# Haochen-Wang409/U2PL

Hardware: AMD Instinct MI355X
Metric: train images/sec at 769x769 (R101-DeepLabv3+) (higher is better)
Workload: dtype f32

## Files before the change

include/u2pl_hip.h:

```cpp
#ifndef U2PL_HIP_H
#define U2PL_HIP_H

#include <stddef.h>
#include <stdint.h>

#ifdef __cplusplus
extern "C" {
#endif

#ifndef __HIP_PLATFORM_AMD__
typedef struct ihipStream_t* hipStream_t;
#endif

#define U2PL_SEL_MAX_SLOTS 8
#define U2PL_SEL_WORD_NVALID 0
#define U2PL_SEL_WORD_NTOTAL 1
#define U2PL_SEL_WORD_VAL 40
#define U2PL_SEL_WORD_THR 56

int u2pl_bilinear_up_f32(const float* in, long sn, long sc, long sh, long sw, int N, int C, int h, int w,
                         float* out_nchw, int H, int W, hipStream_t stream);
int u2pl_bilinear_up_bwd_f32(const float* gout_nchw, int N, int C, int H, int W, float* gin, long sn, long sc,
                             long sh, long sw, int h, int w, hipStream_t stream);
int u2pl_pseudo_label_f32(const float* logits_nchw, int N, int C, int H, int W, float* conf, long long* label,
// ... 136 lines not shown
                          int accumulate, int N, int Hin, int Win, int Cin, int Hout, int Wout, int Cout, int R,
                          int S, int stride, int pad, int dil, hipStream_t stream);
int u2pl_wgrad_set_tr(int on);
int u2pl_im2col_f32(const float* x, long ldx, float* col, int Kp, int N, int Hin, int Win, int Cin, int Hout,
                    int Wout, int R, int S, int stride, int pad, int dil, hipStream_t stream);

size_t u2pl_weight_split3_bytes(int rows, int K, int batch);
int u2pl_weight_split3_f32(const float* w, long zw, int rows, int K, int batch, void* out, hipStream_t stream);
int u2pl_weight_split3_multi_f32(const void* jobs, int njobs, long total, hipStream_t stream);
int u2pl_weight_split3_pad_rows(int rows);
int u2pl_wino_weight_multi_f32(const void* jobs, int njobs, long total, hipStream_t stream);
int u2pl_igemm_ws_stat_blocks(int N, int Hout, int Wout);
int u2pl_igemm_ws_set_persist(int on);
int u2pl_conv2d_fwd_ws_f32(const float* x, long ldx, const void* wsplit, const float* bias, float* y, long ldy, int N,
                           int Hin, int Win, int Cin, int Hout, int Wout, int Cout, int R, int S, int stride, int pad,
                           int dil, hipStream_t stream);
int u2pl_conv2d_fwd_bnstats_ws_f32(const float* x, long ldx, const void* wsplit, const float* bias, float* y, long ldy,
                                   int N, int Hin, int Win, int Cin, int Hout, int Wout, int Cout, int R, int S,
                                   int stride, int pad, int dil, const float* pivot, float* stats_partial,
                                   hipStream_t stream);
int u2pl_conv2d_fwd_bnact_ws_f32(const float* x, long ldx, const void* wsplit, const float* bias, float* y, long ldy, int N,
                                 int Hin, int Win, int Cin, int Hout, int Wout, int Cout, int R, int S, int stride,
                                 int pad, int dil, const float* mean, const float* invstd, const float* gamma,
                                 const float* beta, const float* res, long ldr, int relu, hipStream_t stream);
int u2pl_conv2d_dgrad_ws_f32(const float* dy, long lddy, const void* wTsplit, float* dx, long lddx, int N, int Hin,
                             int Win, int Cin, int Hout, int Wout, int Cout, int R, int S, int stride, int pad, int dil,
                             hipStream_t stream);
int u2pl_gemm_batched_ws_f32(const float* x, long ldx, long zx, const void* wsplit, float* y, long ldy, long zy, long M,
                             int K, int Nn, int batch, hipStream_t stream);

size_t u2pl_weight_split2h_bytes(int rows, int K, int batch);
int u2pl_weight_split2h_f32(const float* w, long zw, int rows, int K, int batch, void* out, void* job_scratch, hipStream_t stream);
int u2pl_weight_split2h_multi_f32(const void* jobs, int njobs, long total, hipStream_t stream);
int u2pl_amax_words(void);
int u2pl_absmax_f32(const float* x, long ld, long M, int C, float* out, int clear, hipStream_t stream);
int u2pl_bn_apply_amax_f32(const float* x, long ldx, const float* mean, const float* invstd, const float* gamma, const float* beta,
                           const float* res, long ldr, int relu, const float* drop, long rows_per_image, float* y, long ldy, long M,
                           int C, float* y_amax, hipStream_t stream);
int u2pl_bn_bwd_apply_amax_f32(const float* dy, long lddy, const float* x, long ldx, const float* y, long ldy, const float* mean,
                               const float* invstd, const float* gamma, const float* drop, long rows_per_image, const double* sums,
                               double count, float* dx, long lddx, float* dres, long lddr, long M, int C, const double* psums,
                               float* gsink, float* bsink, int accumulate, float* dx_amax, float* dres_amax, const float* relu_beta,
                               hipStream_t stream);
int u2pl_bn_bwd_sums_mx_f32(const float* dy, long lddy, const float* x, long ldx, const float* mean, const float* invstd,
                            const float* gamma, const float* beta, const float* drop, long rows_per_image, long M, int C,
                            void* workspace, double* sums, hipStream_t stream);
int u2pl_wino_input_amax_f32(const float* x, long ldx, int N, int H, int W, int C, int dil, int mt, float* V, float* v_amax,
                             hipStream_t stream);
int u2pl_wino_output_bnact_amax_f32(const float* Mb, int N, int H, int W, int O, int dil, int mt, const float* bias, float* y,
                                    long ldy, const float* mean, const float* invstd, const float* gamma, const float* beta,
                                    const float* res, long ldr, int relu, float* y_amax, hipStream_t stream);
int u2pl_wino_gy_amax_f32(const float* gy, long ldg, int N, int H, int W, int O, int dil, int mt, float* Mg, float* mg_amax,
                          hipStream_t stream);
int u2pl_conv2d_fwd_wsh_f32(const float* x, long ldx, const float* x_amax, const void* wsplit, const float* bias, float* y, long ldy,
                            int N, int Hin, int Win, int Cin, int Hout, int Wout, int Cout, int R, int S, int stride, int pad,
                            int dil, hipStream_t stream);
int u2pl_conv2d_fwd_bnstats_wsh_f32(const float* x, long ldx, const float* x_amax, const void* wsplit, const float* bias, float* y,
                                    long ldy, int N, int Hin, int Win, int Cin, int Hout, int Wout, int Cout, int R, int S,
                                    int stride, int pad, int dil, const float* pivot, float* stats_partial, hipStream_t stream);
int u2pl_conv2d_fwd_bnact_wsh_f32(const float* x, long ldx, const float* x_amax, const void* wsplit, const float* bias, float* y,
                                  long ldy, int N, int Hin, int Win, int Cin, int Hout, int Wout, int Cout, int R, int S,
                                  int stride, int pad, int dil, const float* mean, const float* invstd, const float* gamma,
                                  const float* beta, const float* res, long ldr, int relu, float* y_amax, hipStream_t stream);
int u2pl_conv2d_dgrad_wsh_f32(const float* dy, long lddy, const float* dy_amax, const void* wTsplit, float* dx, long lddx, int N,
                              int Hin, int Win, int Cin, int Hout, int Wout, int Cout, int R, int S, int stride, int pad, int dil,
                              hipStream_t stream);
// ... 92 lines not shown
```

u2pl_amd/csrc/igemm_ws.hip:

```cpp
#include <stdlib.h>
#include <type_traits>
#include "common.h"
#include "conv_geom.h"
#include "u2pl_hip.h"

template <int B, int E, class F>
__device__ __forceinline__ void static_for(F&& f) {
    if constexpr (B < E) {
        f(std::integral_constant<int, B>{});
        static_for<B + 1, E>(f);
    }
}

#define WS_ROW_B 64
__host__ __device__ static inline int ws_pad_rows(int rows) { return rows <= 128 ? 128 : (rows + 255) & ~255; }

__global__ void k_weight_split3(const float* __restrict__ w, long zw, unsigned short* __restrict__ out, long zo, int rows,
                                int Np, int K) {
    w += (long)blockIdx.y * zw;
    out += (long)blockIdx.y * zo;
    const int nseg = K / 8;
    const long total = (long)Np * nseg;
    for (long i = blockIdx.x * (long)blockDim.x + threadIdx.x; i < total; i += (long)gridDim.x * blockDim.x) {
        const int sg = (int)(i % nseg), n = (int)(i / nseg);
        float4 v0 = make_float4(0.f, 0.f, 0.f, 0.f), v1 = v0;
        if (n < rows) {
            const float4* src = (const float4*)(w + (long)n * K + sg * 8);
            v0 = src[0];
            v1 = src[1];
        }
        uint2 a0, a1, a2, b0, b1, b2;
        split3_bf16(v0, a0, a1, a2);
        split3_bf16(v1, b0, b1, b2);
        const int c = sg >> 2, s = sg & 3;
        const long base = (((long)c * 3) * Np + n) * 32 + ((s ^ ((n >> 2) & 3)) << 3);
        const long pl = (long)Np * 32;
        *(uint4*)(out + base) = make_uint4(a0.x, a0.y, b0.x, b0.y);
// ... 46 lines not shown
        split3_bf16(v1, b0, b1, b2);
        const int c = sg >> 2, s = sg & 3;
        const long pl = (long)j.Np * 32;
        unsigned short* out = j.out + (long)z * (j.K / 32) * 3 * pl;
        const long base = (((long)c * 3) * j.Np + n) * 32 + ((s ^ ((n >> 2) & 3)) << 3);
        *(uint4*)(out + base) = make_uint4(a0.x, a0.y, b0.x, b0.y);
        *(uint4*)(out + base + pl) = make_uint4(a1.x, a1.y, b1.x, b1.y);
        *(uint4*)(out + base + 2 * pl) = make_uint4(a2.x, a2.y, b2.x, b2.y);
    }
}
U2PL_API int u2pl_weight_split3_multi_f32(const void* jobs, int njobs, long total, hipStream_t stream) {
    if (njobs <= 0 || total <= 0) return njobs == 0 ? 0 : U2PL_EINVAL;
    U2PL_LAUNCH(k_weight_split3_multi, dim3(grid_for(total, 256, 4096)), dim3(256), 0, stream, (const SplitJob*)jobs, njobs, total);
    U2PL_LAUNCH_CHECK();
    return 0;
}
U2PL_API int u2pl_weight_split3_pad_rows(int rows) { return ws_pad_rows(rows); }

U2PL_API size_t u2pl_weight_split3_bytes(int rows, int K, int batch) {
    return (size_t)batch * (K / 32) * 3 * ws_pad_rows(rows) * WS_ROW_B;
}
U2PL_API int u2pl_weight_split3_f32(const float* w, long zw, int rows, int K, int batch, void* out, hipStream_t stream) {
    if (rows <= 0 || K <= 0 || (K % 32) || batch <= 0) return U2PL_EINVAL;
    const int Np = ws_pad_rows(rows);
    const long total = (long)Np * (K / 8);
    dim3 grid(grid_for(total, 256, 2048), batch);
    U2PL_LAUNCH(k_weight_split3, grid, dim3(256), 0, stream, w, zw, (unsigned short*)out,
                (long)(u2pl_weight_split3_bytes(rows, K, 1) / 2), rows, Np, K);
    U2PL_LAUNCH_CHECK();
    return 0;
}

__host__ __device__ static inline size_t ws2_plane_bytes(int Np, int K, int batch) { return (size_t)batch * (K / 32) * 2 * Np * WS_ROW_B; }
__global__ void k_weight_amax_clear(const SplitJob* __restrict__ jobs, int njobs) {
    const int t = blockIdx.x * blockDim.x + threadIdx.x;
    if (t >= njobs) return;
    const SplitJob j = jobs[t];
    unsigned* slot = (unsigned*)((char*)j.out + ws2_plane_bytes(j.Np, j.K, j.batch));
    for (int z = 0; z < ((j.batch + 3) & ~3); ++z) slot[z] = 0u;
}
#define WS_AMAX_SPAN 8192
__global__ __launch_bounds__(256) void k_weight_absmax_multi(const SplitJob* __restrict__ jobs, int njobs, long total) {
    const long begin = (long)blockIdx.x * WS_AMAX_SPAN, end = begin + WS_AMAX_SPAN < total ? begin + WS_AMAX_SPAN : total;
    unsigned* slot = nullptr;
    unsigned m = 0u;
    int lo = 0;
    SplitJob j = jobs[0];
    bool have = false;
    for (long i = begin + threadIdx.x; i < end; i += 256) {
        if (!have || i < j.seg_begin || i >= j.seg_begin + (long)j.batch * j.Np * (j.K / 8)) {
            lo = 0;
            int hi = njobs - 1;
            while (lo < hi) {
                const int mid = (lo + hi + 1) >> 1;
                if (jobs[mid].seg_begin <= i) lo = mid; else hi = mid - 1;
            }
            j = jobs[lo];
            have = true;
        }
        const int nseg = j.K / 8;
        const long per = (long)j.Np * nseg;
        long r = i - j.seg_begin;
        const int z = (int)(r / per);
        r -= (long)z * per;
        unsigned* sl = (unsigned*)((char*)j.out + ws2_plane_bytes(j.Np, j.K, j.batch)) + z;
        if (sl != slot) {
            if (slot && m) atomicMax(slot, m);
            slot = sl;
            m = 0u;
        }
        const int n = (int)(r / nseg), sg = (int)(r % nseg);
        if (n < j.rows) {
            const float4* src = (const float4*)(j.src + ((long)z * j.rows + n) * j.K + sg * 8);
            m = amax_bits4(amax_bits4(m, src[0]), src[1]);
        }
    }
    const unsigned long long key = (unsigned long long)slot;
    const unsigned long long first = (unsigned)__builtin_amdgcn_readfirstlane((int)(unsigned)key) |
                                     ((unsigned long long)(unsigned)__builtin_amdgcn_readfirstlane((int)(unsigned)(key >> 32)) << 32);
    if (__all(key == first)) {
        m = wave_max_u(m);
        if ((threadIdx.x & 63) == 0 && slot && m) atomicMax(slot, m);
    } else if (slot && m) {
        atomicMax(slot, m);
    }
}
__global__ __launch_bounds__(256) void k_weight_split2h_multi(const SplitJob* __restrict__ jobs, int njobs, long total) {
    const long begin = (long)blockIdx.x * WS_AMAX_SPAN, end = begin + WS_AMAX_SPAN < total ? begin + WS_AMAX_SPAN : total;
    SplitJob j = jobs[0];
    bool have = false;
    for (long i = begin + threadIdx.x; i < end; i += 256) {
        if (!have || i < j.seg_begin || i >= j.seg_begin + (long)j.batch * j.Np * (j.K / 8)) {
            int lo = 0, hi = njobs - 1;
            while (lo < hi) {
                const int mid = (lo + hi + 1) >> 1;
                if (jobs[mid].seg_begin <= i) lo = mid; else hi = mid - 1;
            }
            j = jobs[lo];
            have = true;
        }
        const int nseg = j.K / 8;
        const long per = (long)j.Np * nseg;
        long r = i - j.seg_begin;
        const int z = (int)(r / per);
        r -= (long)z * per;
        int sg, n;
        float4 v0 = make_float4(0.f, 0.f, 0.f, 0.f), v1 = v0;
        if (j.kind == 0) {
            sg = (int)(r % nseg);
            n = (int)(r / nseg);
            if (n < j.rows) {
                const float4* src = (const float4*)(j.src + ((long)z * j.rows + n) * j.K + sg * 8);
                v0 = src[0];
                v1 = src[1];
            }
        } else {
            n = (int)(r % j.Np);
            sg = (int)(r / j.Np);
            if (n < j.rows) {
                const int Cout = j.K / j.RS;
                float e[8];
#pragma unroll
                for (int q = 0; q < 8; ++q) {
                    const int k = sg * 8 + q, rs = k / Cout, co = k - rs * Cout;
                    e[q] = j.src[((long)co * j.RS + rs) * j.rows + n];
                }
                v0 = make_float4(e[0], e[1], e[2], e[3]);
                v1 = make_float4(e[4], e[5], e[6], e[7]);
            }
        }
        const unsigned* amax = (const unsigned*)((const char*)j.out + ws2_plane_bytes(j.Np, j.K, j.batch));
        const float sc = split2_scale(split2_exp_bits(amax[z]));
        uint2 a0, a1, b0, b1;
        split2_f16(v0, sc, a0, a1);
        split2_f16(v1, sc, b0, b1);
        const int c = sg >> 2, s_ = sg & 3;
        const long pl = (long)j.Np * 32;
        unsigned short* out = j.out + (long)z * (j.K / 32) * 2 * pl;
        const long base = (((long)c * 2) * j.Np + n) * 32 + ((s_ ^ ((n >> 2) & 3)) << 3);
        *(uint4*)(out + base) = make_uint4(a0.x, a0.y, b0.x, b0.y);
        *(uint4*)(out + base + pl) = make_uint4(a1.x, a1.y, b1.x, b1.y);
    }
}
U2PL_API size_t u2pl_weight_split2h_bytes(int rows, int K, int batch) {
    return ws2_plane_bytes(ws_pad_rows(rows), K, batch) + (((size_t)batch * 4 + 15) & ~(size_t)15);
}
U2PL_API int u2pl_weight_split2h_multi_f32(const void* jobs, int njobs, long total, hipStream_t stream) {
    if (njobs <= 0 || total <= 0) return njobs == 0 ? 0 : U2PL_EINVAL;
    U2PL_LAUNCH(k_weight_amax_clear, dim3(cdiv(njobs, 256)), dim3(256), 0, stream, (const SplitJob*)jobs, njobs);
    U2PL_LAUNCH_CHECK();
    U2PL_LAUNCH(k_weight_absmax_multi, dim3((unsigned)cdiv(total, WS_AMAX_SPAN)), dim3(256), 0, stream, (const SplitJob*)jobs, njobs, total);
    U2PL_LAUNCH_CHECK();
    U2PL_LAUNCH(k_weight_split2h_multi, dim3((unsigned)cdiv(total, WS_AMAX_SPAN)), dim3(256), 0, stream, (const SplitJob*)jobs, njobs, total);
    U2PL_LAUNCH_CHECK();
    return 0;
}
U2PL_API int u2pl_weight_split2h_f32(const float* w, long zw, int rows, int K, int batch, void* out, void* job_scratch, hipStream_t stream) {
    if (rows <= 0 || K <= 0 || (K % 32) || batch <= 0 || !job_scratch) return U2PL_EINVAL;
    if (batch > 1 && zw != (long)rows * K) return U2PL_EINVAL;
    const int Np = ws_pad_rows(rows);
    SplitJob j = {w, (unsigned short*)out, 0, rows, Np, K, 0, 1, batch};
    const long total = (long)batch * Np * (K / 8);
    hipError_t e = hipMemcpyAsync(job_scratch, &j, sizeof j, hipMemcpyHostToDevice, stream);
    if (e != hipSuccess) return (int)e;
    return u2pl_weight_split2h_multi_f32(job_scratch, 1, total, stream);
}
__global__ void k_absmax_rows(const float* __restrict__ x, long ld, long M, int C4, unsigned* __restrict__ out) {
    const long total = M * C4;
    unsigned m = 0;
    for (long i = blockIdx.x * (long)blockDim.x + threadIdx.x; i < total; i += (long)gridDim.x * blockDim.x) {
        const long r = i / C4;
        const int c = (int)(i - r * C4);
        m = amax_bits4(m, *(const float4*)(x + r * ld + c * 4));
    }
    amax_wave_publish(m, out);
}
U2PL_API int u2pl_amax_words(void) { return U2PL_AMAX_WORDS; }
U2PL_API int u2pl_absmax_f32(const float* x, long ld, long M, int C, float* out, int clear, hipStream_t stream) {
    if (M < 0 || C <= 0 || (C & 3) || (ld & 3)) return U2PL_EINVAL;
    if (clear) {
        hipError_t e = hipMemsetAsync(out, 0, (size_t)U2PL_AMAX_WORDS * 4, stream);
        if (e != hipSuccess) return (int)e;
    }
    if (M == 0) return 0;
    U2PL_LAUNCH(k_absmax_rows, dim3(grid_for(M * (C / 4), 512, 2048)), dim3(512), 0, stream, x, ld, M, C / 4, (unsigned*)out);
    U2PL_LAUNCH_CHECK();
    return 0;
}

#ifdef U2PL_WS_STAMPS
__device__ unsigned long long* d_ws_stamps;
static unsigned long long* g_ws_stamps = nullptr;
U2PL_API int u2pl_igemm_ws_set_stamp_buffer(void* p) { g_ws_stamps = (unsigned long long*)p; return 0; }
#endif
template <int TM, int TN, int WM, int WN, bool PW, int ABL = 0, int NP = 3>
__device__ __forceinline__ void igemm_ws_body(
    const float* __restrict__ x, long ldx, const float* __restrict__ x_amax, const unsigned short* __restrict__ ws,
    const unsigned* __restrict__ b_amax, const float* __restrict__ bias,
// ... 807 lines not shown
```

u2pl_amd/csrc/wino.hip:

```cpp
#include "common.h"
#include "u2pl_hip.h"

struct WinoGeom {
    int N, H, W, C, dil, Ty, Tx;
    long tiles;
};

__device__ __forceinline__ float4 f4add(float4 a, float4 b) { return make_float4(a.x + b.x, a.y + b.y, a.z + b.z, a.w + b.w); }
__device__ __forceinline__ float4 f4sub(float4 a, float4 b) { return make_float4(a.x - b.x, a.y - b.y, a.z - b.z, a.w - b.w); }
__device__ __forceinline__ float4 f4mul(float s, float4 a) { return make_float4(s * a.x, s * a.y, s * a.z, s * a.w); }
__device__ __forceinline__ float4 f4axpy(float4 a, float s, float4 b) { return f4add(a, f4mul(s, b)); }

template <int MT> struct WinoT;
template <> struct WinoT<4> {
    static constexpr int A = 6;
    __device__ static __forceinline__ void bt(const float4 (&d)[6], float4 (&r)[6]) {
        const float4 p = f4axpy(d[4], -4.f, d[2]);
        const float4 q = f4axpy(d[3], -4.f, d[1]);
        const float4 s = f4sub(d[4], d[2]);
        const float4 t = f4mul(2.f, f4sub(d[3], d[1]));
        r[0] = f4add(f4axpy(f4mul(4.f, d[0]), -5.f, d[2]), d[4]);
        r[1] = f4add(p, q);
        r[2] = f4sub(p, q);
        r[3] = f4add(s, t);
        r[4] = f4sub(s, t);
        r[5] = f4add(f4axpy(f4mul(4.f, d[1]), -5.f, d[3]), d[5]);
    }
    __device__ static __forceinline__ void at(const float4 (&m)[6], float4 (&y)[4]) {
        const float4 s12 = f4add(m[1], m[2]), d12 = f4sub(m[1], m[2]);
        const float4 s34 = f4add(m[3], m[4]), d34 = f4sub(m[3], m[4]);
        y[0] = f4add(f4add(m[0], s12), s34);
        y[1] = f4axpy(d12, 2.f, d34);
        y[2] = f4axpy(s12, 4.f, s34);
        y[3] = f4add(f4axpy(d12, 8.f, d34), m[5]);
    }
    __device__ static __forceinline__ void av(const float4 (&v)[4], float4 (&r)[6]) {
        const float4 e = f4add(v[0], v[2]), o = f4add(v[1], v[3]);
        const float4 e4 = f4axpy(v[0], 4.f, v[2]), o4 = f4axpy(f4mul(2.f, v[1]), 8.f, v[3]);
        r[0] = v[0];
        r[1] = f4add(e, o);
        r[2] = f4sub(e, o);
        r[3] = f4add(e4, o4);
        r[4] = f4sub(e4, o4);
        r[5] = v[3];
    }
    __device__ static __forceinline__ void gt(const float (&v)[6], float (&r)[3]) {
        const float s12 = v[1] + v[2], s34 = v[3] + v[4];
        r[0] = v[0] * 0.25f - s12 * (1.f / 6.f) + s34 * (1.f / 24.f);
        r[1] = (v[2] - v[1]) * (1.f / 6.f) + (v[3] - v[4]) * (1.f / 12.f);
        r[2] = (s34 - s12) * (1.f / 6.f) + v[5];
    }
    __device__ static __forceinline__ void gg(const float (&g)[3], float (&r)[6]) {
        const float a = (g[0] + g[2]) * (-1.f / 6.f), b = g[1] * (1.f / 6.f);
        const float c = g[0] * (1.f / 24.f) + g[2] * (1.f / 6.f), e = g[1] * (1.f / 12.f);
        r[0] = g[0] * 0.25f;
        r[1] = a - b;
        r[2] = a + b;
        r[3] = c + e;
        r[4] = c - e;
        r[5] = g[2];
    }
};
template <> struct WinoT<2> {
    static constexpr int A = 4;
    __device__ static __forceinline__ void bt(const float4 (&d)[4], float4 (&r)[4]) {
        r[0] = f4sub(d[0], d[2]);
        r[1] = f4add(d[1], d[2]);
        r[2] = f4sub(d[2], d[1]);
        r[3] = f4sub(d[1], d[3]);
    }
    __device__ static __forceinline__ void at(const float4 (&m)[4], float4 (&y)[2]) {
        y[0] = f4add(f4add(m[0], m[1]), m[2]);
        y[1] = f4sub(f4sub(m[1], m[2]), m[3]);
    }
    __device__ static __forceinline__ void av(const float4 (&v)[2], float4 (&r)[4]) {
        r[0] = v[0];
        r[1] = f4add(v[0], v[1]);
        r[2] = f4sub(v[0], v[1]);
        r[3] = f4mul(-1.f, v[1]);
    }
    __device__ static __forceinline__ void gt(const float (&v)[4], float (&r)[3]) {
        r[0] = v[0] + 0.5f * (v[1] + v[2]);
        r[1] = 0.5f * (v[1] - v[2]);
        r[2] = 0.5f * (v[1] + v[2]) + v[3];
    }
    __device__ static __forceinline__ void gg(const float (&g)[3], float (&r)[4]) {
        r[0] = g[0];
        r[1] = 0.5f * ((g[0] + g[2]) + g[1]);
        r[2] = 0.5f * ((g[0] + g[2]) - g[1]);
        r[3] = g[2];
    }
};

__device__ __forceinline__ void tile_coords(const WinoGeom& g, long t, int& n, int& py, int& px, int& ty, int& tx) {
    tx = (int)(t % g.Tx); t /= g.Tx;
    ty = (int)(t % g.Ty); t /= g.Ty;
    px = (int)(t % g.dil); t /= g.dil;
    py = (int)(t % g.dil);
    n = (int)(t / g.dil);
}

template <int MT>
__global__ __launch_bounds__(256) U2PL_HBM_KERNEL void k_wino_input(const float* __restrict__ x, long ldx, unsigned xbytes, WinoGeom g,
                                                    float* __restrict__ V, unsigned* __restrict__ v_amax) {
    constexpr int A = WinoT<MT>::A;
    const int C4 = g.C >> 2;
    long idx = blockIdx.x * (long)blockDim.x + threadIdx.x;
    if (idx >= g.tiles * C4) {
        if (!v_amax) return;
        idx = g.tiles * C4 - 1;
    }
    const int c4 = (int)(idx % C4);
    const long t = idx / C4;
    int n, py, px, ty, tx;
    tile_coords(g, t, n, py, px, ty, tx);
    const __amdgpu_buffer_rsrc_t rx = make_rsrc(x, xbytes);
    const int ldxb = (int)ldx * 4;
    const int iy0 = py + g.dil * (ty * MT - 1), ix0 = px + g.dil * (tx * MT - 1);
    float4 d[A][A];
#pragma unroll
    for (int i = 0; i < A; ++i) {
        const int iy = iy0 + i * g.dil;
        const bool oky = iy >= 0 && iy < g.H;
// ... 13 lines not shown
        WinoT<MT>::bt(col, r);
#pragma unroll
        for (int i = 0; i < A; ++i) d[i][j] = r[i];
    }
    const long comp_stride = g.tiles * (long)g.C;
    float* out = V + t * g.C + c4 * 4;
    unsigned am = 0u;
#pragma unroll
    for (int i = 0; i < A; ++i) {
        float4 r[A];
        WinoT<MT>::bt(d[i], r);
#pragma unroll
        for (int j = 0; j < A; ++j) {
            *(float4*)(out + (long)(i * A + j) * comp_stride) = r[j];
            am = amax_bits4(am, r[j]);
        }
    }
    if (v_amax) amax_wave_publish(am, v_amax);
}

template <int MT>
__device__ __forceinline__ void wino_weight_one(const float* __restrict__ w, int O, int C, int transposed, float* __restrict__ U, long idx) {
    constexpr int A = WinoT<MT>::A;
    const int c = transposed ? (int)(idx / O) : (int)(idx % C), o = transposed ? (int)(idx % O) : (int)(idx / C);
    float gk[3][3];
#pragma unroll
    for (int r = 0; r < 3; ++r)
#pragma unroll
        for (int s = 0; s < 3; ++s) {
            const int rr = transposed ? 2 - r : r, ss = transposed ? 2 - s : s;
            gk[r][s] = w[(((long)o * 3 + rr) * 3 + ss) * C + c];
        }
    float t[A][3];
#pragma unroll
    for (int s = 0; s < 3; ++s) {
        float col[3] = {gk[0][s], gk[1][s], gk[2][s]}, r[A];
        WinoT<MT>::gg(col, r);
#pragma unroll
        for (int i = 0; i < A; ++i) t[i][s] = r[i];
    }
    const long comp_stride = (long)O * C;
    const long base = transposed ? (long)c * O + o : (long)o * C + c;
#pragma unroll
    for (int i = 0; i < A; ++i) {
        float r[A];
        WinoT<MT>::gg(t[i], r);
#pragma unroll
        for (int j = 0; j < A; ++j) U[(long)(i * A + j) * comp_stride + base] = r[j];
    }
}
template <int MT>
__global__ void k_wino_weight(const float* __restrict__ w, int O, int C, int transposed, float* __restrict__ U) {
    const long idx = blockIdx.x * (long)blockDim.x + threadIdx.x;
    if (idx >= (long)O * C) return;
    wino_weight_one<MT>(w, O, C, transposed, U, idx);
}
struct WinoWeightJob { const float* w; float* U; long begin; int O, C, transposed, mt; };
__global__ void k_wino_weight_multi(const WinoWeightJob* __restrict__ jobs, int njobs, long total) {
    for (long i = blockIdx.x * (long)blockDim.x + threadIdx.x; i < total; i += (long)gridDim.x * blockDim.x) {
        int lo = 0, hi = njobs - 1;
        while (lo < hi) {
            const int mid = (lo + hi + 1) >> 1;
            if (jobs[mid].begin <= i) lo = mid; else hi = mid - 1;
        }
        const WinoWeightJob j = jobs[lo];
        if (j.mt == 4) wino_weight_one<4>(j.w, j.O, j.C, j.transposed, j.U, i - j.begin);
        else wino_weight_one<2>(j.w, j.O, j.C, j.transposed, j.U, i - j.begin);
    }
}

template <int MT>
__global__ __launch_bounds__(256) U2PL_HBM_KERNEL void k_wino_output(const float* __restrict__ Mb, WinoGeom g, int O,
                                                     const float* __restrict__ bias, float* __restrict__ y, long ldy,
                                                     float* __restrict__ stats, const float* __restrict__ pivot,
                                                     BnEpi epi) {
    constexpr int A = WinoT<MT>::A;
    __shared__ __attribute__((aligned(16))) float red[2][256][4];
    const int O4 = O >> 2;
    const int tpb = 256 / O4 > 0 ? 256 / O4 : 1;
// ... 323 lines not shown
```

u2pl_amd/nn.py:

```python
import math
import os
import weakref

import torch
import torch.distributed as dist
import torch.nn as nn

from . import _lib
from ._lib import HipError, call, query

from .comm import (COMM_DEBUG, COMM_STATS, _all_reduce, _digest_of, _world, check_comm_sequence, comm_sequence_digest,
                   dist_active, note_collective)
from .layout import _CL, _ws, as_rows, new_act
from .operands import (AMAX_STATS, CONV_H, CONV_WS, PRESPLIT, WEIGHT_EPOCH, _AMAX_POOL, _DerivedCache, _derived, _split_of,
                       _weight_stamp, _ws_ok, amax_of, amax_pool_reset, amax_slot, bump_weight_epoch, invalidate_weights, presplit,
                       set_amax, ws_dgrad, ws_forward, ws_wino)


_WGRAD = {"stream": None, "enabled": os.environ.get("U2PL_NO_WGRAD_STREAM") is None}


def _wgrad_stream():
    if not _WGRAD["enabled"] or _lib.PROFILE is not None:
        return None
    if _WGRAD["stream"] is None:
        _WGRAD["stream"] = torch.cuda.Stream()
    return _WGRAD["stream"]


def wgrad_stream_sync():
    _WGRAD["queued"] = False
    if _WGRAD["stream"] is not None:
        torch.cuda.current_stream().wait_stream(_WGRAD["stream"])
    _lib.SIDE_WORK.discard("wgrad")


def _queue_wgrad_join():
    if not _WGRAD.get("queued"):
        _WGRAD["queued"] = True
        torch.autograd.Variable._execution_engine.queue_callback(wgrad_stream_sync)


def _grad_sink(p):
    return getattr(p, "_u2pl_grad", None)


def _mark_ready(sink):
# ... 1052 lines not shown
```

u2pl_amd/operands.py:

```python
import os

import torch

from . import _lib
from ._lib import HipError, call, query
from .layout import as_rows

WEIGHT_EPOCH = [0]
CONV_WS = {"on": os.environ.get("U2PL_CONV_WS", "1") != "0"}


def bump_weight_epoch(arena=None):
    if arena is None:
        WEIGHT_EPOCH[0] += 1
    else:
        arena.epoch[0] += 1


def _weight_stamp(weight):
    ep = getattr(weight, "_u2pl_epoch", None)
    return (WEIGHT_EPOCH[0], ep[0] if ep is not None else 0, weight._version, weight.data_ptr())


class _DerivedCache(dict):
# ... 100 lines not shown
        ent["spec"] = dict(spec, rows=rows, K=K, batch=batch, h=bool(h))
    return buf


def ws_forward(weight, h=None):
    Cout, Cin, R, S = weight.shape
    return _split_of(weight, "f", Cout, R * S * Cin, 1, lambda: weight, dict(how="plain"), h)


def ws_dgrad(weight, h=None):
    Cout, Cin, R, S = weight.shape

    def src():
        wT = torch.empty(Cin * R * S * Cout, dtype=torch.float32, device=weight.device)
        call("u2pl_weight_transpose_f32", weight, wT, Cout, R * S, Cin)
        return wT
    return _split_of(weight, "d", Cin, R * S * Cout, 1, src, dict(how="transposed", RS=R * S), h)


def ws_wino(weight, transposed, mt, h=None):
    Cout, Cin = weight.shape[:2]
    a2 = (mt + 2) ** 2
    rows, K = (Cin, Cout) if transposed else (Cout, Cin)

    def src():
        U = torch.empty(a2 * Cout * Cin, dtype=torch.float32, device=weight.device)
        call("u2pl_wino_weight_f32", weight, Cout, Cin, int(transposed), mt, U)
        return U
    return _split_of(weight, ("wd" if transposed else "wf") + str(mt), rows, K, a2, src,
                     dict(how="wino", transposed=int(transposed), mt=mt, O=Cout, C=Cin), h)


PRESPLIT = {"on": os.environ.get("U2PL_PRESPLIT", "1") != "0", "tables": {}}


def presplit(params, owner=None):
    import numpy as np
    if not (PRESPLIT["on"] and CONV_WS["on"]):
        return 0
    todo = []
    for w in params:
        cache = w.__dict__.get("_u2pl_derived")
        if not cache:
            continue
        stamp = _weight_stamp(w)
        for kind, ent in cache.items():
            if "spec" in ent and ent["stamp"] is not None and ent["stamp"] != stamp:
                todo.append((w, ent, stamp))
    if not todo:
        return 0
    cur = torch.cuda.current_stream()
    for st in {s_ for _, e, _ in todo for s_ in (list(e["readers"]) + [e["stream"]]) if s_ != cur}:
        cur.wait_stream(st)
    todo.sort(key=lambda t_: bool(t_[1]["spec"].get("h")))
    n_plain = sum(1 for _, e, _ in todo if not e["spec"].get("h"))
    key = tuple((w.data_ptr(), e["buf"].data_ptr(), e["spec"]["how"], bool(e["spec"].get("h"))) for w, e, _ in todo)
    tab = PRESPLIT["tables"].get(id(owner))
    if tab is None or tab["key"] != key:
        dev = todo[0][0].device
        sj = np.zeros(len(todo), dtype=np.dtype([("src", "<u8"), ("out", "<u8"), ("seg", "<i8"), ("rows", "<i4"), ("Np", "<i4"),
                                                 ("K", "<i4"), ("kind", "<i4"), ("RS", "<i4"), ("batch", "<i4")]))
        wino = [(w, e) for w, e, _ in todo if e["spec"]["how"] == "wino"]
        wj = np.zeros(max(len(wino), 1), dtype=np.dtype([("w", "<u8"), ("U", "<u8"), ("begin", "<i8"), ("O", "<i4"), ("C", "<i4"),
                                                         ("tr", "<i4"), ("mt", "<i4")]))
        u_off, acc = {}, 0
        for w, e in wino:
            sp = e["spec"]
            u_off[id(e)] = acc
            acc += sp["batch"] * sp["rows"] * sp["K"]
        scratch = torch.empty(max(acc, 1), dtype=torch.float32, device=dev)
        begin = 0
        for i, (w, e) in enumerate(wino):
            sp = e["spec"]
            wj[i] = (w.data_ptr(), scratch.data_ptr() + 4 * u_off[id(e)], begin, sp["O"], sp["C"], sp["transposed"], sp["mt"])
            begin += sp["O"] * sp["C"]
        seg, segs = 0, [0, 0]
        for i, (w, e, _) in enumerate(todo):
            sp = e["spec"]
            if i == n_plain:
                seg = 0
            Np = query("u2pl_weight_split3_pad_rows", sp["rows"])
            src = scratch.data_ptr() + 4 * u_off[id(e)] if sp["how"] == "wino" else w.data_ptr()
            sj[i] = (src, e["buf"].data_ptr(), seg, sp["rows"], Np, sp["K"], 1 if sp["how"] == "transposed" else 0,
                     sp.get("RS", 1), sp["batch"])
            seg += sp["batch"] * Np * (sp["K"] // 8)
            segs[int(i >= n_plain)] = seg
        sj_dev = torch.from_numpy(sj.view(np.uint8).copy()).to(dev)
        tab = PRESPLIT["tables"][id(owner)] = dict(
            key=key, scratch=scratch, n_plain=n_plain, n_h=len(todo) - n_plain, seg=segs[0], seg_h=segs[1], n_wino=len(wino),
            wino_total=begin, sj=sj_dev, sj_h=sj_dev[n_plain * sj.dtype.itemsize:],
            wj=torch.from_numpy(wj.view(np.uint8).copy()).to(dev))
    if tab["n_wino"]:
        call("u2pl_wino_weight_multi_f32", tab["wj"], tab["n_wino"], tab["wino_total"])
    if tab["n_plain"]:
        call("u2pl_weight_split3_multi_f32", tab["sj"], tab["n_plain"], tab["seg"])
    if tab["n_h"]:
        call("u2pl_weight_split2h_multi_f32", tab["sj_h"], tab["n_h"], tab["seg_h"])
    ev = torch.cuda.Event()
    ev.record(cur)
    for w, e, stamp in todo:
        e["event"], e["stream"], e["stamp"], e["readers"] = ev, cur, stamp, set()
    return len(todo)
```

Baseline: 35.60.

## Fuse Winograd filter transform directly into fp16 split-weight presplit kernels

Winograd-transformed weights that use the two-half split format are now computed directly from the raw 3x3 filters inside the absmax and split kernels. Previously the transformed filters were written to an fp32 scratch buffer and read back. This removes one kernel pass and the scratch-buffer round trip for those layers each time weights are presplit after an optimizer step. The cost is that the filter transform now runs twice, once for absmax and once for the split. The change also adds 32-bit index math for job coordinate decoding and an environment switch to disable the path.

```diff
diff --git a/include/u2pl_hip.h b/include/u2pl_hip.h
--- a/include/u2pl_hip.h
+++ b/include/u2pl_hip.h
@@ -192,6 +192,9 @@
 size_t u2pl_weight_split2h_bytes(int rows, int K, int batch);
 int u2pl_weight_split2h_f32(const float* w, long zw, int rows, int K, int batch, void* out, void* job_scratch, hipStream_t stream);
 int u2pl_weight_split2h_multi_f32(const void* jobs, int njobs, long total, hipStream_t stream);
+int u2pl_wino_direct_pair_span(void);
+int u2pl_weight_split2h_wino_multi_f32(const void* jobs, int njobs, long total, const void* wjobs, int nwjobs, long wpairs,
+                                       long wsegs, hipStream_t stream);
 int u2pl_amax_words(void);
 int u2pl_absmax_f32(const float* x, long ld, long M, int C, float* out, int clear, hipStream_t stream);
 int u2pl_bn_apply_amax_f32(const float* x, long ldx, const float* mean, const float* invstd, const float* gamma, const float* beta,
diff --git a/u2pl_amd/csrc/igemm_ws.hip b/u2pl_amd/csrc/igemm_ws.hip
--- a/u2pl_amd/csrc/igemm_ws.hip
+++ b/u2pl_amd/csrc/igemm_ws.hip
@@ -3,6 +3,7 @@
 #include "common.h"
 #include "conv_geom.h"
 #include "u2pl_hip.h"
+#include "wino_filter.h"
 
 template <int B, int E, class F>
 __device__ __forceinline__ void static_for(F&& f) {
@@ -115,21 +116,49 @@
 }
 
 __host__ __device__ static inline size_t ws2_plane_bytes(int Np, int K, int batch) { return (size_t)batch * (K / 32) * 2 * Np * WS_ROW_B; }
-__global__ void k_weight_amax_clear(const SplitJob* __restrict__ jobs, int njobs) {
+struct WinoDirectJob { const float* w; unsigned short* out; long seg_begin, pair_begin; int O, C, transposed, mt; };
+#define WD_PAIR_SPAN 16384
+__device__ __forceinline__ unsigned* wino_direct_slots(const WinoDirectJob& j) {
+    const int rows = j.transposed ? j.C : j.O, K = j.transposed ? j.O : j.C, a = j.mt + 2;
+    return (unsigned*)((char*)j.out + ws2_plane_bytes(ws_pad_rows(rows), K, a * a));
+}
+__global__ void k_weight_amax_clear(const SplitJob* __restrict__ jobs, int njobs, const WinoDirectJob* __restrict__ wjobs, int nwjobs) {
     const int t = blockIdx.x * blockDim.x + threadIdx.x;
-    if (t >= njobs) return;
-    const SplitJob j = jobs[t];
-    unsigned* slot = (unsigned*)((char*)j.out + ws2_plane_bytes(j.Np, j.K, j.batch));
-    for (int z = 0; z < ((j.batch + 3) & ~3); ++z) slot[z] = 0u;
+    if (t >= njobs + nwjobs) return;
+    unsigned* slot;
+    int batch;
+    if (t < njobs) {
+        const SplitJob j = jobs[t];
+        slot = (unsigned*)((char*)j.out + ws2_plane_bytes(j.Np, j.K, j.batch));
+        batch = j.batch;
+    } else {
+        const WinoDirectJob j = wjobs[t - njobs];
+        slot = wino_direct_slots(j);
+        batch = (j.mt + 2) * (j.mt + 2);
+    }
+    for (int z = 0; z < ((batch + 3) & ~3); ++z) slot[z] = 0u;
+}
+__device__ __forceinline__ void split_job_coords(long r, int Np, int nseg, bool narrow, int& z, int& n, int& sg) {
+    if (narrow) {
+        const unsigned r32 = (unsigned)r, row = r32 / (unsigned)nseg;
+        sg = (int)(r32 - row * (unsigned)nseg);
+        z = (int)(row / (unsigned)Np);
+        n = (int)(row - (unsigned)z * (unsigned)Np);
+    } else {
+        const long row = r / nseg;
+        sg = (int)(r - row * nseg);
+        z = (int)(row / Np);
+        n = (int)(row - (long)z * Np);
+    }
 }
 #define WS_AMAX_SPAN 8192
-__global__ __launch_bounds__(256) void k_weight_absmax_multi(const SplitJob* __restrict__ jobs, int njobs, long total) {
-    const long begin = (long)blockIdx.x * WS_AMAX_SPAN, end = begin + WS_AMAX_SPAN < total ? begin + WS_AMAX_SPAN : total;
+__device__ __forceinline__ void weight_absmax_span(const SplitJob* __restrict__ jobs, int njobs, long total, unsigned blk) {
+    const long begin = (long)blk * WS_AMAX_SPAN, end = begin + WS_AMAX_SPAN < total ? begin + WS_AMAX_SPAN : total;
     unsigned* slot = nullptr;
     unsigned m = 0u;
     int lo = 0;
     SplitJob j = jobs[0];
-    bool have = false;
+    bool have = false, narrow = false;
     for (long i = begin + threadIdx.x; i < end; i += 256) {
         if (!have || i < j.seg_begin || i >= j.seg_begin + (long)j.batch * j.Np * (j.K / 8)) {
             lo = 0;
@@ -140,19 +169,16 @@
             }
             j = jobs[lo];
             have = true;
-        }
-        const int nseg = j.K / 8;
-        const long per = (long)j.Np * nseg;
-        long r = i - j.seg_begin;
-        const int z = (int)(r / per);
-        r -= (long)z * per;
+            narrow = (long)j.batch * j.Np * (j.K / 8) <= 0xffffffffL;
+        }
+        int z, n, sg;
+        split_job_coords(i - j.seg_begin, j.Np, j.K / 8, narrow, z, n, sg);
         unsigned* sl = (unsigned*)((char*)j.out + ws2_plane_bytes(j.Np, j.K, j.batch)) + z;
         if (sl != slot) {
             if (slot && m) atomicMax(slot, m);
             slot = sl;
             m = 0u;
         }
-        const int n = (int)(r / nseg), sg = (int)(r % nseg);
         if (n < j.rows) {
             const float4* src = (const float4*)(j.src + ((long)z * j.rows + n) * j.K + sg * 8);
             m = amax_bits4(amax_bits4(m, src[0]), src[1]);
@@ -167,6 +193,9 @@
     } else if (slot && m) {
         atomicMax(slot, m);
     }
+}
+__global__ __launch_bounds__(256) void k_weight_absmax_multi(const SplitJob* __restrict__ jobs, int njobs, long total) {
+    weight_absmax_span(jobs, njobs, total, blockIdx.x);
 }
 __global__ __launch_bounds__(256) void k_weight_split2h_multi(const SplitJob* __restrict__ jobs, int njobs, long total) {
     const long begin = (long)blockIdx.x * WS_AMAX_SPAN, end = begin + WS_AMAX_SPAN < total ? begin + WS_AMAX_SPAN : total;
@@ -230,7 +259,8 @@
 }
 U2PL_API int u2pl_weight_split2h_multi_f32(const void* jobs, int njobs, long total, hipStream_t stream) {
     if (njobs <= 0 || total <= 0) return njobs == 0 ? 0 : U2PL_EINVAL;
-    U2PL_LAUNCH(k_weight_amax_clear, dim3(cdiv(njobs, 256)), dim3(256), 0, stream, (const SplitJob*)jobs, njobs);
+    U2PL_LAUNCH(k_weight_amax_clear, dim3(cdiv(njobs, 256)), dim3(256), 0, stream, (const SplitJob*)jobs, njobs,
+                (const WinoDirectJob*)nullptr, 0);
     U2PL_LAUNCH_CHECK();
     U2PL_LAUNCH(k_weight_absmax_multi, dim3((unsigned)cdiv(total, WS_AMAX_SPAN)), dim3(256), 0, stream, (const SplitJob*)jobs, njobs, total);
     U2PL_LAUNCH_CHECK();
@@ -247,6 +277,159 @@
     hipError_t e = hipMemcpyAsync(job_scratch, &j, sizeof j, hipMemcpyHostToDevice, stream);
     if (e != hipSuccess) return (int)e;
     return u2pl_weight_split2h_multi_f32(job_scratch, 1, total, stream);
+}
+
+__device__ __forceinline__ WinoDirectJob wino_direct_find(const WinoDirectJob* __restrict__ wjobs, int nwjobs, long at, bool by_pair) {
+    int lo = 0, hi = nwjobs - 1;
+    while (lo < hi) {
+        const int mid = (lo + hi + 1) >> 1;
+        if ((by_pair ? wjobs[mid].pair_begin : wjobs[mid].seg_begin) <= at) lo = mid; else hi = mid - 1;
+    }
+    return wjobs[lo];
+}
+__device__ __forceinline__ void wino_direct_taps(const WinoDirectJob& j, int o, int c, float (&gk)[3][3]) {
+#pragma unroll
+    for (int r = 0; r < 3; ++r)
+#pragma unroll
+        for (int s = 0; s < 3; ++s) {
+            const int rr = j.transposed ? 2 - r : r, ss = j.transposed ? 2 - s : s;
+            gk[r][s] = ldg(j.w + (((long)o * 3 + rr) * 3 + ss) * j.C + c);
+        }
+}
+template <int MT>
+__device__ __forceinline__ void wino_direct_absmax_span(const WinoDirectJob& j, int first, unsigned* s_m) {
+    constexpr int A = WinoG<MT>::A;
+    const int pairs = j.O * j.C, end = first + WD_PAIR_SPAN < pairs ? first + WD_PAIR_SPAN : pairs;
+    unsigned m[A][A];
+#pragma unroll
+    for (int i = 0; i < A; ++i)
+#pragma unroll
+        for (int k = 0; k < A; ++k) m[i][k] = 0u;
+#pragma unroll 1
+    for (int p = first + (int)threadIdx.x; p < end; p += 256) {
+        const int o = p / j.C, c = p - o * j.C;
+        float gk[3][3], t[A][3];
+        wino_direct_taps(j, o, c, gk);
+        wino_filter_cols<MT>(gk, t);
+#pragma unroll
+        for (int i = 0; i < A; ++i) {
+            float r[A];
+            WinoG<MT>::gg(t[i], r);
+#pragma unroll
+            for (int k = 0; k < A; ++k) m[i][k] = amax_bits(m[i][k], r[k]);
+        }
+    }
+    if (threadIdx.x < A * A) s_m[threadIdx.x] = 0u;
+    __syncthreads();
+#pragma unroll
+    for (int i = 0; i < A; ++i)
+#pragma unroll
+        for (int k = 0; k < A; ++k)
+            if (m[i][k]) atomicMax(&s_m[i * A + k], m[i][k]);
+    __syncthreads();
+    if (threadIdx.x < A * A) {
+        const unsigned v = s_m[threadIdx.x];
+        if (v) atomicMax(wino_direct_slots(j) + threadIdx.x, v);
+    }
+}
+__global__ __launch_bounds__(256) void k_weight_absmax_multi_wd(const SplitJob* __restrict__ jobs, int njobs, long total, unsigned nb_plain,
+                                                                const WinoDirectJob* __restrict__ wjobs, int nwjobs) {
+    __shared__ unsigned s_m[36];
+    if (blockIdx.x < nb_plain) {
+        weight_absmax_span(jobs, njobs, total, blockIdx.x);
+        return;
+    }
+    const long at = (long)(blockIdx.x - nb_plain) * WD_PAIR_SPAN;
+    const WinoDirectJob j = wino_direct_find(wjobs, nwjobs, at, true);
+    const long first = at - j.pair_begin;
+    if (first >= (long)j.O * j.C) return;
+    if (j.mt == 4) wino_direct_absmax_span<4>(j, (int)first, s_m);
+    else wino_direct_absmax_span<2>(j, (int)first, s_m);
+}
+template <int MT>
+__device__ __forceinline__ void wino_direct_split_item(const WinoDirectJob& j, int idx) {
+    constexpr int A = WinoG<MT>::A;
+    const int rows = j.transposed ? j.C : j.O, K = j.transposed ? j.O : j.C, Np = ws_pad_rows(rows);
+    if (idx >= Np * (K / 8)) return;
+    const int s_ = idx & 3, rest = idx >> 2, c = rest / Np, n = rest - c * Np, k0 = (c * 4 + s_) * 8;
+    const long pl = (long)Np * 32;
+    const long base = (((long)(k0 >> 5) * 2) * Np + n) * 32 + ((s_ ^ ((n >> 2) & 3)) << 3);
+    if (n >= rows) {
+#pragma unroll
+        for (int z = 0; z < A * A; ++z) {
+            unsigned short* out = j.out + (long)z * (K / 32) * 2 * pl;
+            *(U2PL_GLOBAL u32x4*)(out + base) = u32x4{0u, 0u, 0u, 0u};
+            *(U2PL_GLOBAL u32x4*)(out + base + pl) = u32x4{0u, 0u, 0u, 0u};
+        }
+        return;
+    }
+    const unsigned* amax = wino_direct_slots(j);
+    float sc[A * A];
+#pragma unroll
+    for (int z = 0; z < A * A; ++z) sc[z] = split2_scale(split2_exp_bits(ldg(amax + z)));
+    float gk[8][3][3], t[8][A][3];
+    if (!j.transposed) {
+#pragma unroll
+        for (int r = 0; r < 3; ++r)
+#pragma unroll
+            for (int s = 0; s < 3; ++s) {
+                const u32x4* src = (const u32x4*)(j.w + (((long)n * 3 + r) * 3 + s) * j.C + k0);
+                const u32x4 a = ldg(src), b = ldg(src + 1);
+#pragma unroll
+                for (int q = 0; q < 4; ++q) {
+                    gk[q][r][s] = __uint_as_float(a[q]);
+                    gk[4 + q][r][s] = __uint_as_float(b[q]);
+                }
+            }
+    } else {
+#pragma unroll
+        for (int q = 0; q < 8; ++q) wino_direct_taps(j, k0 + q, n, gk[q]);
+    }
+#pragma unroll
+    for (int q = 0; q < 8; ++q) wino_filter_cols<MT>(gk[q], t[q]);
+#pragma unroll
+    for (int i = 0; i < A; ++i) {
+        float u[8][A];
+#pragma unroll
+        for (int q = 0; q < 8; ++q) WinoG<MT>::gg(t[q][i], u[q]);
+#pragma unroll
+        for (int k = 0; k < A; ++k) {
+            const int z = i * A + k;
+            uint2 a0, a1, b0, b1;
+            split2_f16(make_float4(u[0][k], u[1][k], u[2][k], u[3][k]), sc[z], a0, a1);
+            split2_f16(make_float4(u[4][k], u[5][k], u[6][k], u[7][k]), sc[z], b0, b1);
+            unsigned short* out = j.out + (long)z * (K / 32) * 2 * pl;
+            *(U2PL_GLOBAL u32x4*)(out + base) = u32x4{a0.x, a0.y, b0.x, b0.y};
+            *(U2PL_GLOBAL u32x4*)(out + base + pl) = u32x4{a1.x, a1.y, b1.x, b1.y};
+        }
+    }
+}
+__global__ __launch_bounds__(256) void k_wino_direct_split2h_multi(const WinoDirectJob* __restrict__ wjobs, int nwjobs) {
+    const long at = (long)blockIdx.x * 256;
+    const WinoDirectJob j = wino_direct_find(wjobs, nwjobs, at, false);
+    const int idx = (int)(at - j.seg_begin) + (int)threadIdx.x;
+    if (j.mt == 4) wino_direct_split_item<4>(j, idx);
+    else wino_direct_split_item<2>(j, idx);
+}
+U2PL_API int u2pl_wino_direct_pair_span(void) { return WD_PAIR_SPAN; }
+U2PL_API int u2pl_weight_split2h_wino_multi_f32(const void* jobs, int njobs, long total, const void* wjobs, int nwjobs, long wpairs,
+                                                long wsegs, hipStream_t stream) {
+    if (njobs < 0 || nwjobs <= 0 || (njobs > 0) != (total > 0) || wpairs <= 0 || wpairs % WD_PAIR_SPAN || wsegs <= 0 || wsegs % 256)
+        return U2PL_EINVAL;
+    const unsigned nb_plain = (unsigned)cdiv(total, WS_AMAX_SPAN);
+    U2PL_LAUNCH(k_weight_amax_clear, dim3(cdiv(njobs + nwjobs, 256)), dim3(256), 0, stream, (const SplitJob*)jobs, njobs,
+                (const WinoDirectJob*)wjobs, nwjobs);
+    U2PL_LAUNCH_CHECK();
+    U2PL_LAUNCH(k_weight_absmax_multi_wd, dim3(nb_plain + (unsigned)(wpairs / WD_PAIR_SPAN)), dim3(256), 0, stream,
+                (const SplitJob*)jobs, njobs, total, nb_plain, (const WinoDirectJob*)wjobs, nwjobs);
+    U2PL_LAUNCH_CHECK();
+    if (njobs) {
+        U2PL_LAUNCH(k_weight_split2h_multi, dim3(nb_plain), dim3(256), 0, stream, (const SplitJob*)jobs, njobs, total);
+        U2PL_LAUNCH_CHECK();
+    }
+    U2PL_LAUNCH(k_wino_direct_split2h_multi, dim3((unsigned)(wsegs / 256)), dim3(256), 0, stream, (const WinoDirectJob*)wjobs, nwjobs);
+    U2PL_LAUNCH_CHECK();
+    return 0;
 }
 __global__ void k_absmax_rows(const float* __restrict__ x, long ld, long M, int C4, unsigned* __restrict__ out) {
     const long total = M * C4;
diff --git a/u2pl_amd/csrc/wino.hip b/u2pl_amd/csrc/wino.hip
--- a/u2pl_amd/csrc/wino.hip
+++ b/u2pl_amd/csrc/wino.hip
@@ -1,5 +1,6 @@
 #include "common.h"
 #include "u2pl_hip.h"
+#include "wino_filter.h"
 
 struct WinoGeom {
     int N, H, W, C, dil, Ty, Tx;
@@ -50,16 +51,6 @@
         r[1] = (v[2] - v[1]) * (1.f / 6.f) + (v[3] - v[4]) * (1.f / 12.f);
         r[2] = (s34 - s12) * (1.f / 6.f) + v[5];
     }
-    __device__ static __forceinline__ void gg(const float (&g)[3], float (&r)[6]) {
-        const float a = (g[0] + g[2]) * (-1.f / 6.f), b = g[1] * (1.f / 6.f);
-        const float c = g[0] * (1.f / 24.f) + g[2] * (1.f / 6.f), e = g[1] * (1.f / 12.f);
-        r[0] = g[0] * 0.25f;
-        r[1] = a - b;
-        r[2] = a + b;
-        r[3] = c + e;
-        r[4] = c - e;
-        r[5] = g[2];
-    }
 };
 template <> struct WinoT<2> {
     static constexpr int A = 4;
@@ -83,12 +74,6 @@
         r[0] = v[0] + 0.5f * (v[1] + v[2]);
         r[1] = 0.5f * (v[1] - v[2]);
         r[2] = 0.5f * (v[1] + v[2]) + v[3];
-    }
-    __device__ static __forceinline__ void gg(const float (&g)[3], float (&r)[4]) {
-        r[0] = g[0];
-        r[1] = 0.5f * ((g[0] + g[2]) + g[1]);
-        r[2] = 0.5f * ((g[0] + g[2]) - g[1]);
-        r[3] = g[2];
     }
 };
 
@@ -168,19 +153,13 @@
             gk[r][s] = w[(((long)o * 3 + rr) * 3 + ss) * C + c];
         }
     float t[A][3];
-#pragma unroll
-    for (int s = 0; s < 3; ++s) {
-        float col[3] = {gk[0][s], gk[1][s], gk[2][s]}, r[A];
-        WinoT<MT>::gg(col, r);
-#pragma unroll
-        for (int i = 0; i < A; ++i) t[i][s] = r[i];
-    }
+    wino_filter_cols<MT>(gk, t);
     const long comp_stride = (long)O * C;
     const long base = transposed ? (long)c * O + o : (long)o * C + c;
 #pragma unroll
     for (int i = 0; i < A; ++i) {
         float r[A];
-        WinoT<MT>::gg(t[i], r);
+        WinoG<MT>::gg(t[i], r);
 #pragma unroll
         for (int j = 0; j < A; ++j) U[(long)(i * A + j) * comp_stride + base] = r[j];
     }
diff --git a/u2pl_amd/csrc/wino_filter.h b/u2pl_amd/csrc/wino_filter.h
--- /dev/null
+++ b/u2pl_amd/csrc/wino_filter.h
@@ -0,0 +1,37 @@
+#pragma once
+
+template <int MT> struct WinoG;
+template <> struct WinoG<4> {
+    static constexpr int A = 6;
+    __device__ static __forceinline__ void gg(const float (&g)[3], float (&r)[6]) {
+        const float a = (g[0] + g[2]) * (-1.f / 6.f), b = g[1] * (1.f / 6.f);
+        const float c = g[0] * (1.f / 24.f) + g[2] * (1.f / 6.f), e = g[1] * (1.f / 12.f);
+        r[0] = g[0] * 0.25f;
+        r[1] = a - b;
+        r[2] = a + b;
+        r[3] = c + e;
+        r[4] = c - e;
+        r[5] = g[2];
+    }
+};
+template <> struct WinoG<2> {
+    static constexpr int A = 4;
+    __device__ static __forceinline__ void gg(const float (&g)[3], float (&r)[4]) {
+        r[0] = g[0];
+        r[1] = 0.5f * ((g[0] + g[2]) + g[1]);
+        r[2] = 0.5f * ((g[0] + g[2]) - g[1]);
+        r[3] = g[2];
+    }
+};
+
+template <int MT>
+__device__ __forceinline__ void wino_filter_cols(const float (&gk)[3][3], float (&t)[WinoG<MT>::A][3]) {
+    constexpr int A = WinoG<MT>::A;
+#pragma unroll
+    for (int s = 0; s < 3; ++s) {
+        float col[3] = {gk[0][s], gk[1][s], gk[2][s]}, r[A];
+        WinoG<MT>::gg(col, r);
+#pragma unroll
+        for (int i = 0; i < A; ++i) t[i][s] = r[i];
+    }
+}
diff --git a/u2pl_amd/nn.py b/u2pl_amd/nn.py
--- a/u2pl_amd/nn.py
+++ b/u2pl_amd/nn.py
@@ -12,7 +12,7 @@
 from .comm import (COMM_DEBUG, COMM_STATS, _all_reduce, _digest_of, _world, check_comm_sequence, comm_sequence_digest,
                    dist_active, note_collective)
 from .layout import _CL, _ws, as_rows, new_act
-from .operands import (AMAX_STATS, CONV_H, CONV_WS, PRESPLIT, WEIGHT_EPOCH, _AMAX_POOL, _DerivedCache, _derived, _split_of,
+from .operands import (AMAX_STATS, CONV_H, CONV_WS, PRESPLIT, WEIGHT_EPOCH, WINO_DIRECT, _AMAX_POOL, _DerivedCache, _derived, _split_of,
                        _weight_stamp, _ws_ok, amax_of, amax_pool_reset, amax_slot, bump_weight_epoch, invalidate_weights, presplit,
                        set_amax, ws_dgrad, ws_forward, ws_wino)
 
diff --git a/u2pl_amd/operands.py b/u2pl_amd/operands.py
--- a/u2pl_amd/operands.py
+++ b/u2pl_amd/operands.py
@@ -156,6 +156,7 @@
 
 
 PRESPLIT = {"on": os.environ.get("U2PL_PRESPLIT", "1") != "0", "tables": {}}
+WINO_DIRECT = {"on": os.environ.get("U2PL_NO_WINO_DIRECT", "0") != "1"}
 
 
 def presplit(params, owner=None):
@@ -176,30 +177,35 @@
     cur = torch.cuda.current_stream()
     for st in {s_ for _, e, _ in todo for s_ in (list(e["readers"]) + [e["stream"]]) if s_ != cur}:
         cur.wait_stream(st)
-    todo.sort(key=lambda t_: bool(t_[1]["spec"].get("h")))
+
+    def direct(e):
+        return WINO_DIRECT["on"] and e["spec"]["how"] == "wino" and bool(e["spec"].get("h"))
+    todo.sort(key=lambda t_: 2 if direct(t_[1]) else int(bool(t_[1]["spec"].get("h"))))
     n_plain = sum(1 for _, e, _ in todo if not e["spec"].get("h"))
-    key = tuple((w.data_ptr(), e["buf"].data_ptr(), e["spec"]["how"], bool(e["spec"].get("h"))) for w, e, _ in todo)
+    n_wd = sum(1 for _, e, _ in todo if direct(e))
+    key = tuple((w.data_ptr(), e["buf"].data_ptr(), e["spec"]["how"], bool(e["spec"].get("h")), direct(e)) for w, e, _ in todo)
     tab = PRESPLIT["tables"].get(id(owner))
     if tab is None or tab["key"] != key:
         dev = todo[0][0].device
-        sj = np.zeros(len(todo), dtype=np.dtype([("src", "<u8"), ("out", "<u8"), ("seg", "<i8"), ("rows", "<i4"), ("Np", "<i4"),
-                                                 ("K", "<i4"), ("kind", "<i4"), ("RS", "<i4"), ("batch", "<i4")]))
-        wino = [(w, e) for w, e, _ in todo if e["spec"]["how"] == "wino"]
-        wj = np.zeros(max(len(wino), 1), dtype=np.dtype([("w", "<u8"), ("U", "<u8"), ("begin", "<i8"), ("O", "<i4"), ("C", "<i4"),
+        split = todo[:len(todo) - n_wd]
+        sj = np.zeros(len(split), dtype=np.dtype([("src", "<u8"), ("out", "<u8"), ("seg", "<i8"), ("rows", "<i4"), ("Np", "<i4"),
+                                                  ("K", "<i4"), ("kind", "<i4"), ("RS", "<i4"), ("batch", "<i4")]))
+        wino = [(w, e) for w, e, _ in split if e["spec"]["how"] == "wino"]
+        wj = np.zeros(len(wino), dtype=np.dtype([("w", "<u8"), ("U", "<u8"), ("begin", "<i8"), ("O", "<i4"), ("C", "<i4"),
                                                          ("tr", "<i4"), ("mt", "<i4")]))
         u_off, acc = {}, 0
         for w, e in wino:
             sp = e["spec"]
             u_off[id(e)] = acc
             acc += sp["batch"] * sp["rows"] * sp["K"]
-        scratch = torch.empty(max(acc, 1), dtype=torch.float32, device=dev)
+        scratch = torch.empty(acc, dtype=torch.float32, device=dev) if acc else None
         begin = 0
         for i, (w, e) in enumerate(wino):
             sp = e["spec"]
             wj[i] = (w.data_ptr(), scratch.data_ptr() + 4 * u_off[id(e)], begin, sp["O"], sp["C"], sp["transposed"], sp["mt"])
             begin += sp["O"] * sp["C"]
         seg, segs = 0, [0, 0]
-        for i, (w, e, _) in enumerate(todo):
+        for i, (w, e, _) in enumerate(split):
             sp = e["spec"]
             if i == n_plain:
                 seg = 0
@@ -209,16 +215,29 @@
                      sp.get("RS", 1), sp["batch"])
             seg += sp["batch"] * Np * (sp["K"] // 8)
             segs[int(i >= n_plain)] = seg
+        dj = np.zeros(n_wd, dtype=np.dtype([("w", "<u8"), ("out", "<u8"), ("seg", "<i8"), ("pair", "<i8"), ("O", "<i4"),
+                                                    ("C", "<i4"), ("tr", "<i4"), ("mt", "<i4")]))
+        span = query("u2pl_wino_direct_pair_span") if n_wd else 1
+        wsegs = wpairs = 0
+        for i, (w, e, _) in enumerate(todo[len(split):]):
+            sp = e["spec"]
+            dj[i] = (w.data_ptr(), e["buf"].data_ptr(), wsegs, wpairs, sp["O"], sp["C"], sp["transposed"], sp["mt"])
+            wsegs += query("u2pl_weight_split3_pad_rows", sp["rows"]) * (sp["K"] // 8)
+            wpairs += -(-sp["O"] * sp["C"] // span) * span
         sj_dev = torch.from_numpy(sj.view(np.uint8).copy()).to(dev)
         tab = PRESPLIT["tables"][id(owner)] = dict(
-            key=key, scratch=scratch, n_plain=n_plain, n_h=len(todo) - n_plain, seg=segs[0], seg_h=segs[1], n_wino=len(wino),
+            key=key, scratch=scratch, n_plain=n_plain, n_h=len(split) - n_plain, seg=segs[0], seg_h=segs[1], n_wino=len(wino),
             wino_total=begin, sj=sj_dev, sj_h=sj_dev[n_plain * sj.dtype.itemsize:],
-            wj=torch.from_numpy(wj.view(np.uint8).copy()).to(dev))
+            wj=torch.from_numpy(wj.view(np.uint8).copy()).to(dev) if len(wino) else None,
+            n_wd=n_wd, wsegs=wsegs, wpairs=wpairs, dj=torch.from_numpy(dj.view(np.uint8).copy()).to(dev) if n_wd else None)
     if tab["n_wino"]:
         call("u2pl_wino_weight_multi_f32", tab["wj"], tab["n_wino"], tab["wino_total"])
     if tab["n_plain"]:
         call("u2pl_weight_split3_multi_f32", tab["sj"], tab["n_plain"], tab["seg"])
-    if tab["n_h"]:
+    if tab["n_wd"]:
+        call("u2pl_weight_split2h_wino_multi_f32", tab["sj_h"], tab["n_h"], tab["seg_h"], tab["dj"], tab["n_wd"], tab["wpairs"],
+             tab["wsegs"])
+    elif tab["n_h"]:
         call("u2pl_weight_split2h_multi_f32", tab["sj_h"], tab["n_h"], tab["seg_h"])
     ev = torch.cuda.Event()
     ev.record(cur)
```

Result: faster. 35.97, median of 6 (+1.1%).
